# scroll-tech/scroll-prover

Measured on NVIDIA H100. Metric: chunk-proof wall-sec (degree-26 SRS: k=20+24+25 replay), lower is better.
Workload: dtype u32x8 (254-bit Montgomery integers)

## Files before the change

### scroll-prover_b200/csrc/api.cu

```cuda
#include <stdlib.h>

#include <new>

#include "common.cuh"
#include "ec.cuh"

namespace b200zk {
int32_t g1_generator_mul_run(b200zk_ctx* ctx, const Fr* scalars, uint64_t n, Affine* out);
int32_t poly_ew(b200zk_ctx* ctx, int op, Fr* r, const Fr* a, const Fr* b, const Fr& s, uint64_t n);
int32_t eval_poly(b200zk_ctx* ctx, const Fr* poly, uint64_t n, const Fr& x, Fr* out_dev);
int32_t batch_invert(b200zk_ctx* ctx, Fr* data, uint64_t n);
int32_t inner_product(b200zk_ctx* ctx, const Fr* a, const Fr* b, uint64_t n, Fr* out_dev);
int32_t kate_division(b200zk_ctx* ctx, Fr* q, const Fr* a, uint64_t n, const Fr& b);
int32_t g1_fft_run(b200zk_ctx* ctx, const void* in, bool from_jac, void* out, bool to_jac, uint32_t log_n, const Fr& omega,
                   const Fr* scale);
int32_t field_op(b200zk_ctx* ctx, int field, int op, void* r, const void* a, const void* b, uint64_t n);
}

using namespace b200zk;

#define CHECK_CTX(ctx) \
    if (!(ctx)) return B200ZK_E_INVALID

extern "C" {

int32_t b200zk_ctx_create(const int* devices, int n_devices, b200zk_ctx** out) {
    if (!out) return B200ZK_E_INVALID;
    *out = nullptr;
    if (n_devices != 1 && !(n_devices == 0 && devices == nullptr)) return B200ZK_E_UNSUPPORTED;
    int dev = (devices && n_devices == 1) ? devices[0] : 0;
    int count = 0;
    if (cudaGetDeviceCount(&count) != cudaSuccess || count == 0) {
        (void)cudaGetLastError();
        return B200ZK_E_CUDA;
    }
    if (dev < 0 || dev >= count) return B200ZK_E_INVALID;
    if (cudaSetDevice(dev) != cudaSuccess) return B200ZK_E_CUDA;
    b200zk_ctx* ctx = new (std::nothrow) b200zk_ctx();
    if (!ctx) return B200ZK_E_OOM;
    ctx->device = dev;
    cudaDeviceProp prop;
    if (cudaGetDeviceProperties(&prop, dev) == cudaSuccess) ctx->sm_count = prop.multiProcessorCount;
    if (cudaStreamCreateWithFlags(&ctx->stream, cudaStreamNonBlocking) != cudaSuccess) {
        delete ctx;
        return B200ZK_E_CUDA;
    }
    ctx->own_stream = true;
    if (const char* e = getenv("B200ZK_OVERLAP")) ctx->overlap = atoi(e);
    if (const char* e = getenv("B200ZK_ACC_L")) ctx->msm_acc_l = (uint32_t)atoi(e);
    if (const char* e = getenv("B200ZK_SCATTER_SWEEPS")) ctx->msm_scatter_sweeps = (uint32_t)atoi(e);
    if (cudaMalloc(&ctx->msm_adds_dev, 8) == cudaSuccess) cudaMemset(ctx->msm_adds_dev, 0, 8);
    else ctx->msm_adds_dev = nullptr;
    *out = ctx;
    return B200ZK_OK;
}

int32_t b200zk_ctx_destroy(b200zk_ctx* ctx) {
    CHECK_CTX(ctx);
    cudaSetDevice(ctx->device);
    cudaStreamSynchronize(ctx->stream);
    comm_destroy(ctx);
    for (Scratch* s : {&ctx->ntt_work, &ctx->stage_in, &ctx->stage_out, &ctx->msm_work, &ctx->misc})
        if (s->p) cudaFree(s->p);
    for (auto& t : ctx->tables) cudaFree(t.dev);
    if (ctx->pinned) cudaFreeHost(ctx->pinned);
    if (ctx->msm_adds_dev) cudaFree(ctx->msm_adds_dev);
    for (Scratch* s : {&ctx->colstage[0], &ctx->colstage[1], &ctx->col_coeff, &ctx->col_ext, &ctx->col_commits})
        if (s->p) cudaFree(s->p);
    for (int i = 0; i < 2; ++i) {
        if (ctx->ev_copied[i]) cudaEventDestroy(ctx->ev_copied[i]);
        if (ctx->ev_used[i]) cudaEventDestroy(ctx->ev_used[i]);
        if (ctx->ev_used_aux[i]) cudaEventDestroy(ctx->ev_used_aux[i]);
    }
    if (ctx->ev_fork) cudaEventDestroy(ctx->ev_fork);
    if (ctx->ev_join) cudaEventDestroy(ctx->ev_join);
    if (ctx->copy_stream) cudaStreamDestroy(ctx->copy_stream);
    if (ctx->aux_stream) cudaStreamDestroy(ctx->aux_stream);
    if (ctx->own_stream && ctx->stream) cudaStreamDestroy(ctx->stream);
    delete ctx;
    return B200ZK_OK;
}

const char* b200zk_last_error(const b200zk_ctx* ctx) { return ctx ? ctx->err.c_str() : "null context"; }

int32_t b200zk_ctx_set_stream(b200zk_ctx* ctx, void* cuda_stream) {
    CHECK_CTX(ctx);
    Guard g(ctx);
    B2_CUDA(ctx, cudaStreamSynchronize(ctx->stream));
    if (cuda_stream == nullptr) {
        if (!ctx->own_stream) {
            B2_CUDA(ctx, cudaStreamCreateWithFlags(&ctx->stream, cudaStreamNonBlocking));
            ctx->own_stream = true;
        }
        return B200ZK_OK;
    }
    if (ctx->own_stream && ctx->stream) cudaStreamDestroy(ctx->stream);
    ctx->stream = (cudaStream_t)cuda_stream;
    ctx->own_stream = false;
    return B200ZK_OK;
}

int32_t b200zk_ctx_synchronize(b200zk_ctx* ctx) {
    CHECK_CTX(ctx);
    Guard g(ctx);
    B2_CUDA(ctx, cudaStreamSynchronize(ctx->stream));
    return B200ZK_OK;
}

int32_t b200zk_ctx_launch_count(const b200zk_ctx* ctx, uint64_t* out) {
    if (!ctx || !out) return B200ZK_E_INVALID;
    *out = ctx->launches;
    return B200ZK_OK;
}

int32_t b200zk_buf_alloc(b200zk_ctx* ctx, uint64_t bytes, void** out_dev) {
    CHECK_CTX(ctx);
    if (!out_dev) return fail(ctx, B200ZK_E_INVALID, "buf_alloc: null out");
    Guard g(ctx);
    *out_dev = nullptr;
    cudaError_t e = cudaMalloc(out_dev, bytes ? bytes : 1);
    if (e != cudaSuccess) {
        (void)cudaGetLastError();
        return fail(ctx, B200ZK_E_OOM, "buf_alloc(%llu) failed: %s", (unsigned long long)bytes, cudaGetErrorString(e));
    }
    return B200ZK_OK;
}
int32_t b200zk_buf_free(b200zk_ctx* ctx, void* dev) {
    CHECK_CTX(ctx);
    Guard g(ctx);
    if (!dev) return B200ZK_OK;
    B2_CUDA(ctx, cudaStreamSynchronize(ctx->stream));
    B2_CUDA(ctx, cudaFree(dev));
    return B200ZK_OK;
// ... 612 lines not shown
```

### scroll-prover_b200/csrc/common.cuh

```cuda
#pragma once
#include <cuda_runtime.h>
#include <stdarg.h>
#include <stdint.h>
#include <stdio.h>
#include <string.h>

#include <mutex>
#include <string>
#include <vector>

#include "../../include/b200zk.h"
#include "ff.cuh"

namespace b200zk {

struct TwiddleTable {
    Fr omega;
    uint32_t log_n;
    Fr* dev;
};

enum ProfKey { PROF_NTT_PASS = 0, PROF_NTT_TABLE, PROF_MSM_COUNT, PROF_MSM_SCAN, PROF_MSM_SCATTER, PROF_MSM_ACCUM,
               PROF_MSM_COMBINE, PROF_MSM_REDUCE, PROF_MSM_FINISH, PROF_POLY, PROF_NKEYS };
static const char* const PROF_NAMES[PROF_NKEYS] = {"ntt_pass", "ntt_table", "msm_count", "msm_scan", "msm_scatter",
                                                   "msm_accumulate", "msm_combine", "msm_reduce", "msm_finish", "poly"};
struct ProfSpan {
    int key;
    cudaEvent_t e0, e1;
};

struct Scratch {
    void* p = nullptr;
    size_t cap = 0;
};

}

struct b200zk_srs {
    b200zk_ctx* ctx;
    void* dev_bases;
    uint64_t n;
    uint32_t tag;
    uint32_t pre_c;
    uint32_t pre_W;
};

struct b200zk_ctx {
    int device = 0;
    cudaStream_t stream = nullptr;
    bool own_stream = true;
    std::recursive_mutex mu;
    std::string err;
    uint64_t launches = 0;
    int sm_count = 132;
    b200zk::Scratch ntt_work, stage_in, stage_out, msm_work, misc;
    void* pinned = nullptr;
    size_t pinned_cap = 0;
    std::vector<b200zk::TwiddleTable> tables;
    cudaStream_t copy_stream = nullptr;
    cudaStream_t aux_stream = nullptr;
    cudaEvent_t ev_used_aux[2] = {nullptr, nullptr}, ev_fork = nullptr, ev_join = nullptr;
    int overlap = 1;
    b200zk::Scratch colstage[2], col_coeff, col_ext, col_commits;
    cudaEvent_t ev_copied[2] = {nullptr, nullptr}, ev_used[2] = {nullptr, nullptr};
    bool profiling = false;
    std::vector<b200zk::ProfSpan> prof_open;
    std::vector<cudaEvent_t> prof_pool;
    double prof_ms[b200zk::PROF_NKEYS] = {0};
    uint64_t prof_cnt[b200zk::PROF_NKEYS] = {0};
    uint32_t msm_window = 0;
    uint32_t msm_scatter_sweeps = 0;
    uint32_t msm_acc_l = 0;
    int srs_precompute = 1;
    unsigned long long* msm_adds_dev = nullptr;
    uint32_t last_c = 0, last_windows = 0;
    uint64_t last_adds = 0;
    uint32_t smem_optin = 0;
    void* nccl_comm = nullptr;
    void* comm_buf = nullptr;
    int comm_rank = 0, comm_world = 1;
};

namespace b200zk {

inline int32_t fail(b200zk_ctx* ctx, int32_t code, const char* fmt, ...) {
    char buf[512];
    va_list ap;
    va_start(ap, fmt);
    vsnprintf(buf, sizeof buf, fmt, ap);
    va_end(ap);
    if (ctx) ctx->err = buf;
    return code;
}

#define B2_CUDA(ctx, call)                                                                                   \
    do {                                                                                                     \
        cudaError_t e__ = (call);                                                                            \
        if (e__ != cudaSuccess)                                                                              \
            return ::b200zk::fail(ctx, e__ == cudaErrorMemoryAllocation ? B200ZK_E_OOM : B200ZK_E_CUDA,      \
                                  "%s failed: %s (%s:%d)", #call, cudaGetErrorString(e__), __FILE__, __LINE__); \
    } while (0)

#define B2_TRY(expr)                    \
    do {                                \
        int32_t rc__ = (expr);          \
        if (rc__ != B200ZK_OK) return rc__; \
    } while (0)

#define B2_LAUNCH_CHECK(ctx)                 \
    do {                                     \
        (ctx)->launches++;                   \
        B2_CUDA(ctx, cudaGetLastError());    \
    } while (0)

inline cudaEvent_t prof_event(b200zk_ctx* ctx) {
    if (!ctx->prof_pool.empty()) {
        cudaEvent_t e = ctx->prof_pool.back();
        ctx->prof_pool.pop_back();
        return e;
    }
    cudaEvent_t e = nullptr;
    cudaEventCreate(&e);
    return e;
}
struct ProfScope {
    b200zk_ctx* ctx;
    ProfSpan sp;
    bool on;
    ProfScope(b200zk_ctx* c, int key) : ctx(c), on(c->profiling) {
        if (!on) return;
        sp.key = key;
        sp.e0 = prof_event(c);
        sp.e1 = prof_event(c);
        cudaEventRecord(sp.e0, c->stream);
    }
    ~ProfScope() {
        if (!on) return;
        cudaEventRecord(sp.e1, ctx->stream);
        ctx->prof_open.push_back(sp);
    }
};
inline void prof_resolve(b200zk_ctx* ctx) {
    for (auto& sp : ctx->prof_open) {
        float ms = 0;
        if (cudaEventSynchronize(sp.e1) == cudaSuccess && cudaEventElapsedTime(&ms, sp.e0, sp.e1) == cudaSuccess) {
            ctx->prof_ms[sp.key] += ms;
            ctx->prof_cnt[sp.key] += 1;
        }
        ctx->prof_pool.push_back(sp.e0);
        ctx->prof_pool.push_back(sp.e1);
    }
    ctx->prof_open.clear();
}

// ... 128 lines not shown
```

### scroll-prover_b200/csrc/msm.cu

```cuda
#include "common.cuh"
#include "ec.cuh"

namespace b200zk {

static constexpr uint32_t PART_INVALID = 0x1fffffffu;
static constexpr uint32_t PART_GIANT = 0x20000000u;
static constexpr uint32_t PART_STARTS = 0x80000000u;
static constexpr uint32_t PART_ENDS = 0x40000000u;
static constexpr int MSM_MAX_BATCH = 32;
static constexpr int ACC_L_DEFAULT = 256;

struct MsmPlan {
    uint32_t c, W, B;
    uint32_t Ws;
    uint32_t batch;
    uint64_t stride;
    uint64_t NB;
};

struct MsmCols {
    const Fr* p[MSM_MAX_BATCH];
};

__device__ __forceinline__ void ld_affine(const Affine* p, Fq& x, Fq& y) {
    const uint4* q = reinterpret_cast<const uint4*>(p);
    uint4 a = __ldg(q), b = __ldg(q + 1), c = __ldg(q + 2), d = __ldg(q + 3);
    x.l.v[0] = a.x; x.l.v[1] = a.y; x.l.v[2] = a.z; x.l.v[3] = a.w;
    x.l.v[4] = b.x; x.l.v[5] = b.y; x.l.v[6] = b.z; x.l.v[7] = b.w;
    y.l.v[0] = c.x; y.l.v[1] = c.y; y.l.v[2] = c.z; y.l.v[3] = c.w;
    y.l.v[4] = d.x; y.l.v[5] = d.y; y.l.v[6] = d.z; y.l.v[7] = d.w;
}

__global__ void __launch_bounds__(256) msm_count(MsmCols cols, uint64_t n, MsmPlan pl, uint32_t* hist, uint32_t* digits_all) {
    const uint32_t col = blockIdx.y;
    const Fr* scalars = cols.p[0];
#pragma unroll
    for (int q = 1; q < MSM_MAX_BATCH; ++q)
        if (q == (int)col) scalars = cols.p[q];
    uint32_t* digits = digits_all + (uint64_t)col * pl.W * n;
    uint32_t* hist_c = hist + (uint64_t)col * pl.Ws * pl.B;
    uint64_t stride = (uint64_t)gridDim.x * blockDim.x;
    for (uint64_t i = (uint64_t)blockIdx.x * blockDim.x + threadIdx.x; i < n; i += stride) {
        Fr s = scalars[i];
        if (s.is_zero()) {
            for (uint32_t w = 0; w < pl.W; ++w) digits[(uint64_t)w * n + i] = 0;
            continue;
        }
        s = s.from_mont();
        uint32_t l[8];
#pragma unroll
        for (int k = 0; k < 8; ++k) l[k] = s.l.v[k];
        const uint32_t c = pl.c, mask = (1u << c) - 1, half = 1u << (c - 1);
        uint32_t carry = 0;
        for (uint32_t w = 0; w < pl.W; ++w) {
            uint32_t v = (l[0] & mask) + carry;
#pragma unroll
            for (int k = 0; k < 7; ++k) l[k] = __funnelshift_r(l[k], l[k + 1], c);
            l[7] >>= c;
            uint32_t enc;
            if (v > half) {
                enc = (1u << c) - v;
                carry = 1;
                if (enc) enc |= 0x80000000u;
            } else {
                enc = v;
                carry = 0;
            }
            digits[(uint64_t)w * n + i] = enc;
            if (enc) atomicAdd(&hist_c[(pl.Ws == 1 ? 0ull : (uint64_t)w * pl.B) + (enc & 0x7fffffffu) - 1], 1u);
        }
    }
}

__global__ void __launch_bounds__(256) msm_scatter(const uint32_t* __restrict__ digits, uint64_t n, MsmPlan pl,
                                                   uint32_t* cursor, uint32_t* entries, const uint32_t* __restrict__ total_entries,
                                                   uint32_t sweep, uint32_t max_sweeps) {
    uint32_t eff = 1;
    if (max_sweeps > 1) {
        uint64_t bytes = 4ull * (*total_entries);
        eff = (uint32_t)((bytes + (1ull << 28) - 1) >> 28);
        eff = eff < 1 ? 1 : (eff > max_sweeps ? max_sweeps : eff);
    }
    if (sweep >= eff) return;
    const uint32_t b_lo = eff == 3 ? (pl.B / 3) * sweep : (pl.B / eff) * sweep;
    const uint32_t b_hi = (sweep + 1 == eff) ? pl.B : (eff == 3 ? (pl.B / 3) * (sweep + 1) : (pl.B / eff) * (sweep + 1));
    const uint32_t cw = blockIdx.y;
    const uint32_t col = cw / pl.W, w = cw - col * pl.W;
    const uint32_t* dg = digits + (uint64_t)cw * n;
    uint32_t* cur = cursor + ((uint64_t)col * pl.Ws + (pl.Ws == 1 ? 0u : w)) * pl.B;
    const uint32_t woff = (uint32_t)((uint64_t)w * pl.stride);
    uint64_t stride = (uint64_t)gridDim.x * blockDim.x;
    for (uint64_t i = (uint64_t)blockIdx.x * blockDim.x + threadIdx.x; i < n; i += stride) {
        uint32_t d = dg[i];
        if (!d) continue;
        uint32_t bk = (d & 0x7fffffffu) - 1;
        if (bk < b_lo || bk >= b_hi) continue;
        uint32_t pos = atomicAdd(&cur[bk], 1u);
        entries[pos] = ((uint32_t)i + woff) | (d & 0x80000000u);
    }
}

static constexpr int SCAN_TPB = 256, SCAN_ITEMS = 16, SCAN_TILE = SCAN_TPB * SCAN_ITEMS;

__device__ __forceinline__ uint32_t block_exclusive_scan(uint32_t v, uint32_t* total) {
    __shared__ uint32_t warp_sums[SCAN_TPB / 32];
    uint32_t lane = threadIdx.x & 31, wid = threadIdx.x >> 5;
    uint32_t x = v;
#pragma unroll
    for (int o = 1; o < 32; o <<= 1) {
        uint32_t y = __shfl_up_sync(0xffffffffu, x, o);
        if (lane >= (uint32_t)o) x += y;
    }
    if (lane == 31) warp_sums[wid] = x;
    __syncthreads();
    if (wid == 0) {
        uint32_t s = (lane < SCAN_TPB / 32) ? warp_sums[lane] : 0;
#pragma unroll
        for (int o = 1; o < 32; o <<= 1) {
            uint32_t y = __shfl_up_sync(0xffffffffu, s, o);
            if (lane >= (uint32_t)o) s += y;
        }
        if (lane < SCAN_TPB / 32) warp_sums[lane] = s;
    }
    __syncthreads();
    uint32_t warp_off = wid ? warp_sums[wid - 1] : 0;
    *total = warp_sums[SCAN_TPB / 32 - 1];
    uint32_t r = warp_off + x - v;
    __syncthreads();
    return r;
}

__global__ void __launch_bounds__(SCAN_TPB) scan_tile_sums(const uint32_t* in, uint64_t n, uint32_t* tile_sums) {
    uint64_t base = (uint64_t)blockIdx.x * SCAN_TILE + (uint64_t)threadIdx.x * SCAN_ITEMS;
    uint32_t s = 0;
#pragma unroll
    for (int k = 0; k < SCAN_ITEMS; ++k)
        if (base + k < n) s += in[base + k];
    uint32_t total;
    block_exclusive_scan(s, &total);
    if (threadIdx.x == 0) tile_sums[blockIdx.x] = total;
}
__global__ void __launch_bounds__(SCAN_TPB) scan_tile_offsets(uint32_t* tile_sums, uint32_t ntiles, uint32_t* grand_total,
                                                              unsigned long long* running) {
    uint32_t carry = 0;
    for (uint32_t base = 0; base < ntiles; base += SCAN_TPB) {
        uint32_t i = base + threadIdx.x;
        uint32_t v = i < ntiles ? tile_sums[i] : 0, total;
        uint32_t ex = block_exclusive_scan(v, &total);
        if (i < ntiles) tile_sums[i] = carry + ex;
        carry += total;
    }
    if (threadIdx.x == 0) {
        *grand_total = carry;
        if (running) atomicAdd(running, (unsigned long long)carry);
    }
}
__global__ void __launch_bounds__(SCAN_TPB) scan_apply(const uint32_t* in, uint64_t n, const uint32_t* tile_offs, uint32_t* out,
                                                     uint32_t* out2) {
    uint64_t base = (uint64_t)blockIdx.x * SCAN_TILE + (uint64_t)threadIdx.x * SCAN_ITEMS;
    uint32_t v[SCAN_ITEMS], s = 0;
#pragma unroll
    for (int k = 0; k < SCAN_ITEMS; ++k) {
        v[k] = (base + k < n) ? in[base + k] : 0;
        s += v[k];
    }
    uint32_t total;
    uint32_t off = block_exclusive_scan(s, &total) + tile_offs[blockIdx.x];
#pragma unroll
    for (int k = 0; k < SCAN_ITEMS; ++k) {
        if (base + k < n) {
            out[base + k] = off;
            out2[base + k] = off;
        }
        off += v[k];
    }
}

__device__ __forceinline__ void st_xyzz(XYZZ* p, const XYZZ& v) {
    uint4* q = reinterpret_cast<uint4*>(p);
    const Fq* f = &v.x;
#pragma unroll
    for (int k = 0; k < 4; ++k) {
        q[2 * k] = make_uint4(f[k].l.v[0], f[k].l.v[1], f[k].l.v[2], f[k].l.v[3]);
        q[2 * k + 1] = make_uint4(f[k].l.v[4], f[k].l.v[5], f[k].l.v[6], f[k].l.v[7]);
    }
}
__device__ __forceinline__ XYZZ ld_xyzz(const XYZZ* p) {
    const uint4* q = reinterpret_cast<const uint4*>(p);
    XYZZ v;
    Fq* f = &v.x;
#pragma unroll
    for (int k = 0; k < 4; ++k) {
        uint4 a = q[2 * k], b = q[2 * k + 1];
        f[k].l.v[0] = a.x; f[k].l.v[1] = a.y; f[k].l.v[2] = a.z; f[k].l.v[3] = a.w;
        f[k].l.v[4] = b.x; f[k].l.v[5] = b.y; f[k].l.v[6] = b.z; f[k].l.v[7] = b.w;
    }
    return v;
}

__global__ void __launch_bounds__(256, 2)
msm_accumulate(const Affine* __restrict__ bases, const uint32_t* __restrict__ entries, const uint32_t* __restrict__ offsets,
               uint64_t NB, XYZZ* __restrict__ buckets, uint32_t* __restrict__ part_id, XYZZ* __restrict__ part_val,
               uint64_t nthreads, uint32_t* __restrict__ giant_flag, uint32_t ACC_L) {
    uint64_t tau = (uint64_t)blockIdx.x * blockDim.x + threadIdx.x;
    if (tau >= nthreads) return;
    const uint32_t M = offsets[NB];
    const uint32_t BIG_BUCKET = 4 * ACC_L;
    uint64_t start = tau * ACC_L;
    part_id[2 * tau] = PART_INVALID;
    part_id[2 * tau + 1] = PART_INVALID;
    if (start >= M) return;
    uint32_t end = (start + ACC_L < M) ? (uint32_t)(start + ACC_L) : M;
    uint64_t lo = 0, hi = NB;
    while (hi - lo > 1) {
        uint64_t mid = (lo + hi) >> 1;
        if (offsets[mid] <= start) lo = mid; else hi = mid;
    }
    uint32_t b = (uint32_t)lo;
    uint32_t bucket_start = offsets[b], bucket_end = offsets[b + 1];
    bool run_starts = (bucket_start == (uint32_t)start);
    uint32_t slot = 0;
    XYZZ acc = XYZZ::identity();
    uint32_t pos = (uint32_t)start;
    while (true) {
        bool at_end = (pos == end);
        if (at_end || pos == bucket_end) {
            bool run_ends = (pos == bucket_end);
            if (run_starts && run_ends) {
                st_xyzz(buckets + b, acc);
            } else {
                uint32_t giant = (bucket_end - bucket_start > BIG_BUCKET) ? PART_GIANT : 0u;
                if (giant) *giant_flag = 1u;
                part_id[2 * tau + slot] = b | giant | (run_starts ? PART_STARTS : 0u) | (run_ends ? PART_ENDS : 0u);
                st_xyzz(part_val + 2 * tau + slot, acc);
                ++slot;
            }
            if (at_end) break;
            acc = XYZZ::identity();
            bucket_start = pos;
            do { ++b; bucket_end = offsets[b + 1]; } while (bucket_end == pos);
            run_starts = true;
        }
        uint32_t e = entries[pos];
        Fq px, py;
        ld_affine(bases + (e & 0x7fffffffu), px, py);
        if (!(px.is_zero() && py.is_zero())) {
            if (e & 0x80000000u) py = py.neg();
            xyzz_madd(acc, px, py);
        }
        ++pos;
    }
}

__global__ void __launch_bounds__(128) msm_combine_heads(const uint32_t* __restrict__ part_id, const XYZZ* __restrict__ part_val,
                                                         uint64_t nrec, XYZZ* __restrict__ buckets) {
    uint64_t r = (uint64_t)blockIdx.x * blockDim.x + threadIdx.x;
    if (r >= nrec) return;
    uint32_t id = part_id[r];
    if ((id & PART_INVALID) == PART_INVALID || (id & PART_GIANT) || !(id & PART_STARTS)) return;
// ... 195 lines not shown
}

static uint32_t pick_window(uint64_t n) {
    if (n < 32) return n < 4 ? 2 : 4;
    double best = 1e300;
    uint32_t bc = 8;
    for (uint32_t c = 5; c <= 23; ++c) {
        uint32_t W = 254 / c + 1;
        if ((double)n * W >= 4.0e9) continue;
        double cost = (double)n * W * 10.0 + (double)W * (double)(1ull << c) * 40.0 + (double)W * 4096.0;
        if (cost < best) {
            best = cost;
            bc = c;
        }
    }
    return bc;
}

static size_t align_up(size_t v, size_t a) { return (v + a - 1) / a * a; }

__global__ void __launch_bounds__(128) srs_shift_kernel(const Affine* __restrict__ in, Affine* __restrict__ out, uint64_t n, uint32_t c) {
    uint64_t i = (uint64_t)blockIdx.x * blockDim.x + threadIdx.x;
    if (i >= n) return;
    Affine a = in[i];
    XYZZ p = xyzz_from_affine(a);
    for (uint32_t d = 0; d < c; ++d) p = xyzz_dbl(p);
    out[i] = xyzz_to_affine(p);
}

static uint32_t pick_window_precomputed(uint64_t n) {
    double best = 1e300;
    uint32_t bc = 10;
    for (uint32_t c = 8; c <= 23; ++c) {
        uint32_t W = 254 / c + 1;
        if ((double)n * W >= 2.0e9) continue;
        double cost = (double)n * W * 10.0 + (double)(1ull << c) * 40.0;
        if (cost < best) {
            best = cost;
            bc = c;
        }
    }
    return bc;
}

static int32_t srs_precompute_run(b200zk_ctx* ctx, Affine* tables, uint64_t n, uint32_t c, uint32_t W) {
    for (uint32_t w = 1; w < W; ++w) {
        srs_shift_kernel<<<(uint32_t)((n + 127) / 128), 128, 0, ctx->stream>>>(tables + (uint64_t)(w - 1) * n, tables + (uint64_t)w * n, n, c);
        B2_LAUNCH_CHECK(ctx);
    }
    return B200ZK_OK;
}

static uint32_t msm_max_batch(uint64_t n, uint32_t pre_c) {
    uint32_t c = pre_c ? pre_c : pick_window(n);
    uint64_t per_col = (n ? n : 1) * (254 / c + 1);
    uint64_t b = (1ull << 28) / per_col;
    return (uint32_t)(b < 1 ? 1 : (b > MSM_MAX_BATCH ? MSM_MAX_BATCH : b));
}

static int32_t msm_run_batch(b200zk_ctx* ctx, const Affine* bases, const Fr* const* cols, uint32_t batch, uint64_t n, Jacobian* out_dev,
                             uint32_t pre_c, uint64_t pre_stride) {
    if (n >= (1ull << 31)) return fail(ctx, B200ZK_E_UNSUPPORTED, "msm: n = %llu >= 2^31", (unsigned long long)n);
    if (batch < 1 || batch > (uint32_t)MSM_MAX_BATCH) return fail(ctx, B200ZK_E_INVALID, "msm: batch %u out of range [1,%d]", batch, MSM_MAX_BATCH);
    MsmPlan pl;
    pl.c = pre_c ? pre_c : (ctx->msm_window ? ctx->msm_window : pick_window(n));
    if (pl.c < 2 || pl.c > 24) return fail(ctx, B200ZK_E_INVALID, "msm: window %u out of range [2,24]", pl.c);
    pl.W = 254 / pl.c + 1;
    pl.B = 1u << (pl.c - 1);
    pl.Ws = pre_c ? 1 : pl.W;
    pl.batch = batch;
    pl.stride = pre_c ? pre_stride : 0;
    pl.NB = (uint64_t)batch * pl.Ws * pl.B;
    uint64_t max_entries = n * pl.W * batch;
    if (max_entries >= 0xffffffffull) return fail(ctx, B200ZK_E_UNSUPPORTED, "msm: n*W*batch too large for window %u", pl.c);
    MsmCols colp;
    for (int q = 0; q < MSM_MAX_BATCH; ++q) colp.p[q] = cols[q < (int)batch ? q : 0];
    ctx->last_c = pl.c;
    ctx->last_windows = pl.W;
    ctx->last_adds = n * pl.W;

    const uint32_t ACC_L = ctx->msm_acc_l ? ctx->msm_acc_l : (uint32_t)ACC_L_DEFAULT;
    uint64_t nthreads = (max_entries + ACC_L - 1) / ACC_L;
    if (nthreads == 0) nthreads = 1;
    uint32_t ntiles = (uint32_t)((pl.NB + SCAN_TILE - 1) / SCAN_TILE);
    size_t off = 0;
    auto carve = [&](size_t bytes) { size_t o = off; off = align_up(off + bytes, 256); return o; };
    size_t o_hist = carve(4 * (pl.NB + 1)), o_offs = carve(4 * (pl.NB + 1)), o_cursor = carve(4 * (pl.NB + 1));
    size_t o_tiles = carve(4 * (size_t)(ntiles + 1));
    size_t o_flag = carve(256);
    size_t o_entries = carve(4 * (max_entries + 4));
    size_t o_digits = carve(4 * (max_entries + 4));
    size_t o_buckets = carve(sizeof(XYZZ) * pl.NB);
    size_t o_pid = carve(4 * 2 * nthreads), o_pval = carve(sizeof(XYZZ) * 2 * nthreads);
    uint64_t nthreads2 = (2 * nthreads + COMBINE_LR - 1) / COMBINE_LR;
    size_t o_pid2 = carve(4 * 2 * nthreads2), o_pval2 = carve(sizeof(XYZZ) * 2 * nthreads2);
    const uint32_t kc = pl.c / 2;
    const uint32_t red_cols = 1u << kc, red_rows = pl.B >> kc;
    const uint32_t sets = batch * pl.Ws;
    size_t red_len = (size_t)sets * (red_rows + red_cols);
    uint32_t q_max = 0;
    while ((1u << q_max) < (red_rows > red_cols ? red_rows : red_cols)) ++q_max;
    size_t o_gr = carve(sizeof(XYZZ) * red_len), o_sums = carve(sizeof(XYZZ) * 2 * (q_max + 1) * sets);
    B2_TRY(scratch_reserve(ctx, ctx->msm_work, off));
    char* base = (char*)ctx->msm_work.p;
    uint32_t* hist = (uint32_t*)(base + o_hist);
    uint32_t* offsets = (uint32_t*)(base + o_offs);
    uint32_t* cursor = (uint32_t*)(base + o_cursor);
    uint32_t* tiles = (uint32_t*)(base + o_tiles);
    uint32_t* giant_flag = (uint32_t*)(base + o_flag);
    uint32_t* entries = (uint32_t*)(base + o_entries);
    uint32_t* digits = (uint32_t*)(base + o_digits);
    uint32_t* pid2 = (uint32_t*)(base + o_pid2);
    XYZZ* pval2 = (XYZZ*)(base + o_pval2);
    XYZZ* buckets = (XYZZ*)(base + o_buckets);
    uint32_t* pid = (uint32_t*)(base + o_pid);
    XYZZ* pval = (XYZZ*)(base + o_pval);
    XYZZ* grpR = (XYZZ*)(base + o_gr);
    XYZZ* red_sums = (XYZZ*)(base + o_sums);

    cudaStream_t st = ctx->stream;
    B2_CUDA(ctx, cudaMemsetAsync(hist, 0, 4 * (pl.NB + 1), st));
    B2_CUDA(ctx, cudaMemsetAsync(giant_flag, 0, 4, st));
    B2_CUDA(ctx, cudaMemsetAsync(buckets, 0, sizeof(XYZZ) * pl.NB, st));
    uint32_t sblocks = (uint32_t)ctx->sm_count * 8;
    if (n) {
        uint64_t want = (n + 255) / 256;
        uint32_t per_col = (sblocks + batch - 1) / batch;
        uint32_t blocks = (uint32_t)(want < per_col ? want : per_col);
        {
            ProfScope ps_(ctx, PROF_MSM_COUNT);
            msm_count<<<dim3(blocks, batch), 256, 0, st>>>(colp, n, pl, hist, digits);
        }
        B2_LAUNCH_CHECK(ctx);
    }
    {
        ProfScope ps_(ctx, PROF_MSM_SCAN);
        scan_tile_sums<<<ntiles, SCAN_TPB, 0, st>>>(hist, pl.NB, tiles);
        B2_LAUNCH_CHECK(ctx);
        scan_tile_offsets<<<1, SCAN_TPB, 0, st>>>(tiles, ntiles, offsets + pl.NB, ctx->msm_adds_dev);
        B2_LAUNCH_CHECK(ctx);
        scan_apply<<<ntiles, SCAN_TPB, 0, st>>>(hist, pl.NB, tiles, offsets, cursor);
        B2_LAUNCH_CHECK(ctx);
    }
    if (n) {
        {
            ProfScope ps_(ctx, PROF_MSM_SCATTER);
            uint64_t want = (n + 1023) / 1024;
            uint32_t blocks = (uint32_t)(want < 0x7fffffffull ? (want ? want : 1) : 0x7fffffffull);
            {
                uint32_t sweeps = 1;
                if (pl.Ws == 1 && batch == 1) {
                    uint64_t region = 200ull << 20;
                    sweeps = (uint32_t)((4 * max_entries + region - 1) / region);
                    if (sweeps < 1) sweeps = 1;
                    if (sweeps > 4) sweeps = 4;
                    if (ctx->msm_scatter_sweeps) sweeps = ctx->msm_scatter_sweeps;
                }
                for (uint32_t sw = 0; sw < sweeps; ++sw) {
                    uint32_t bx = blocks;
                    if (sw > 0) {
                        uint32_t lean = (uint32_t)ctx->sm_count * 32u / (batch * pl.W) + 1;
                        if (lean < bx) bx = lean;
                    }
                    msm_scatter<<<dim3(bx, batch * pl.W), 256, 0, st>>>(digits, n, pl, cursor, entries, offsets + pl.NB, sw, sweeps);
                    if (sw + 1 < sweeps) B2_LAUNCH_CHECK(ctx);
                }
            }
        }
        B2_LAUNCH_CHECK(ctx);
        uint32_t ablocks = (uint32_t)((nthreads + 255) / 256);
        {
            ProfScope ps_(ctx, PROF_MSM_ACCUM);
            msm_accumulate<<<ablocks, 256, 0, st>>>(bases, entries, offsets, pl.NB, buckets, pid, pval, nthreads, giant_flag, ACC_L);
        }
        B2_LAUNCH_CHECK(ctx);
        {
            ProfScope ps_(ctx, PROF_MSM_COMBINE);
            uint64_t nrec = 2 * nthreads;
            msm_combine_heads<<<(uint32_t)((nrec + 127) / 128), 128, 0, st>>>(pid, pval, nrec, buckets);
            B2_LAUNCH_CHECK(ctx);
            uint32_t *in_id = pid, *out_id = pid2;
            XYZZ *in_val = pval, *out_val = pval2;
            while (nrec > 2048) {
                uint64_t nt = (nrec + COMBINE_LR - 1) / COMBINE_LR;
                msm_combine_level<<<(uint32_t)((nt + 127) / 128), 128, 0, st>>>(in_id, in_val, nrec, buckets, out_id, out_val, nt, giant_flag);
                B2_LAUNCH_CHECK(ctx);
                nrec = 2 * nt;
                uint32_t* ti = in_id; in_id = out_id; out_id = ti;
                XYZZ* tv = in_val; in_val = out_val; out_val = tv;
            }
            msm_combine_final<<<(uint32_t)((nrec + 127) / 128), 128, 0, st>>>(in_id, in_val, nrec, buckets, giant_flag);
            B2_LAUNCH_CHECK(ctx);
        }
    }
    {
        ProfScope ps_(ctx, PROF_MSM_REDUCE);
        msm_rowcol_sums<<<dim3(red_rows + red_cols, sets), RED_T, 0, st>>>(buckets, pl.B, kc, grpR);
        B2_LAUNCH_CHECK(ctx);
        msm_bit_sums<<<dim3(q_max + 1, 2, sets), RED_T, 0, st>>>(grpR, pl.B, kc, q_max, red_sums);
        B2_LAUNCH_CHECK(ctx);
        msm_finish<<<batch, 64, 0, st>>>(pl, kc, q_max, red_sums, out_dev);
        B2_LAUNCH_CHECK(ctx);
    }
    return B200ZK_OK;
}

int32_t msm_bases(b200zk_ctx* ctx, const Affine* bases, const Fr* scalars, uint64_t n, Jacobian* out_dev) {
    return msm_run_batch(ctx, bases, &scalars, 1, n, out_dev, 0, 0);
}

int32_t srs_init(b200zk_ctx* ctx, b200zk_srs* s, const void* g1_affine) {
    const uint64_t n = s->n;
    s->dev_bases = nullptr;
    s->pre_c = 0;
    s->pre_W = 1;
    size_t bytes = sizeof(Affine) * (n ? n : 1);
    if (ctx->srs_precompute && n >= (1ull << 16)) {
        uint32_t c = pick_window_precomputed(n), W = 254 / c + 1;
        size_t free_b = 0, total_b = 0;
        if (cudaMemGetInfo(&free_b, &total_b) == cudaSuccess && (double)bytes * W < 0.35 * (double)free_b) {
            s->pre_c = c;
            s->pre_W = W;
            bytes *= W;
        }
    }
    cudaError_t e = cudaMalloc(&s->dev_bases, bytes);
    if (e != cudaSuccess) {
        (void)cudaGetLastError();
        s->dev_bases = nullptr;
        return fail(ctx, B200ZK_E_OOM, "srs_register: cudaMalloc(%zu) failed", bytes);
    }
    cudaMemcpyKind kind = is_device_ptr(g1_affine) ? cudaMemcpyDeviceToDevice : cudaMemcpyHostToDevice;
    e = n ? cudaMemcpyAsync(s->dev_bases, g1_affine, sizeof(Affine) * n, kind, ctx->stream) : cudaSuccess;
    if (e == cudaSuccess) e = cudaStreamSynchronize(ctx->stream);
    if (e != cudaSuccess) {
        srs_free(s);
        return fail(ctx, B200ZK_E_CUDA, "srs_register: upload failed: %s", cudaGetErrorString(e));
    }
    if (s->pre_c) {
        int32_t rc = srs_precompute_run(ctx, (Affine*)s->dev_bases, n, s->pre_c, s->pre_W);
        if (rc == B200ZK_OK && cudaStreamSynchronize(ctx->stream) != cudaSuccess) rc = B200ZK_E_CUDA;
        if (rc != B200ZK_OK) {
            srs_free(s);
            return fail(ctx, rc, "srs_register: precomputation failed");
        }
    }
    return B200ZK_OK;
}

void srs_free(b200zk_srs* s) {
    if (s->dev_bases) cudaFree(s->dev_bases);
    s->dev_bases = nullptr;
// ... 30 lines not shown
```

Baseline: 4.536.

## Replace MSM global-atomic histogram and scatter with two-level tiled bucket sort

Swaps the global-atomic bucket histogram and the multi-sweep scatter in the MSM for a two-level bin sort. Per-tile shared-memory counts go into a bin-by-tile matrix, which is prefix-scanned. Entries are placed into coarse bins in a staging buffer, then each bin is sorted into final buckets in shared memory with dynamic bin assignment. The goal is to cut contended global atomics and random scattered writes. In exchange it adds extra passes, a staging buffer, heavy shared-memory use, and a new failure path when no plan fits.

```diff
diff --git a/scroll-prover_b200/csrc/api.cu b/scroll-prover_b200/csrc/api.cu
--- a/scroll-prover_b200/csrc/api.cu
+++ b/scroll-prover_b200/csrc/api.cu
@@ -48,7 +48,6 @@
     ctx->own_stream = true;
     if (const char* e = getenv("B200ZK_OVERLAP")) ctx->overlap = atoi(e);
     if (const char* e = getenv("B200ZK_ACC_L")) ctx->msm_acc_l = (uint32_t)atoi(e);
-    if (const char* e = getenv("B200ZK_SCATTER_SWEEPS")) ctx->msm_scatter_sweeps = (uint32_t)atoi(e);
     if (cudaMalloc(&ctx->msm_adds_dev, 8) == cudaSuccess) cudaMemset(ctx->msm_adds_dev, 0, 8);
     else ctx->msm_adds_dev = nullptr;
     *out = ctx;
diff --git a/scroll-prover_b200/csrc/common.cuh b/scroll-prover_b200/csrc/common.cuh
--- a/scroll-prover_b200/csrc/common.cuh
+++ b/scroll-prover_b200/csrc/common.cuh
@@ -69,7 +69,6 @@
     double prof_ms[b200zk::PROF_NKEYS] = {0};
     uint64_t prof_cnt[b200zk::PROF_NKEYS] = {0};
     uint32_t msm_window = 0;
-    uint32_t msm_scatter_sweeps = 0;
     uint32_t msm_acc_l = 0;
     int srs_precompute = 1;
     unsigned long long* msm_adds_dev = nullptr;
diff --git a/scroll-prover_b200/csrc/msm.cu b/scroll-prover_b200/csrc/msm.cu
--- a/scroll-prover_b200/csrc/msm.cu
+++ b/scroll-prover_b200/csrc/msm.cu
@@ -31,16 +31,106 @@
     y.l.v[4] = d.x; y.l.v[5] = d.y; y.l.v[6] = d.z; y.l.v[7] = d.w;
 }
 
-__global__ void __launch_bounds__(256) msm_count(MsmCols cols, uint64_t n, MsmPlan pl, uint32_t* hist, uint32_t* digits_all) {
-    const uint32_t col = blockIdx.y;
+static constexpr int SCAN_TPB = 256, SCAN_ITEMS = 16, SCAN_TILE = SCAN_TPB * SCAN_ITEMS;
+
+template <int TPB = SCAN_TPB>
+__device__ __forceinline__ uint32_t block_exclusive_scan(uint32_t v, uint32_t* total) {
+    static_assert(TPB % 32 == 0 && TPB <= 1024, "one warp scans the warp sums");
+    __shared__ uint32_t warp_sums[TPB / 32];
+    uint32_t lane = threadIdx.x & 31, wid = threadIdx.x >> 5;
+    uint32_t x = v;
+#pragma unroll
+    for (int o = 1; o < 32; o <<= 1) {
+        uint32_t y = __shfl_up_sync(0xffffffffu, x, o);
+        if (lane >= (uint32_t)o) x += y;
+    }
+    if (lane == 31) warp_sums[wid] = x;
+    __syncthreads();
+    if (wid == 0) {
+        uint32_t s = (lane < TPB / 32) ? warp_sums[lane] : 0;
+#pragma unroll
+        for (int o = 1; o < 32; o <<= 1) {
+            uint32_t y = __shfl_up_sync(0xffffffffu, s, o);
+            if (lane >= (uint32_t)o) s += y;
+        }
+        if (lane < TPB / 32) warp_sums[lane] = s;
+    }
+    __syncthreads();
+    uint32_t warp_off = wid ? warp_sums[wid - 1] : 0;
+    *total = warp_sums[TPB / 32 - 1];
+    uint32_t r = warp_off + x - v;
+    __syncthreads();
+    return r;
+}
+
+__global__ void __launch_bounds__(SCAN_TPB) scan_tile_sums(const uint32_t* in, uint64_t n, uint32_t* tile_sums) {
+    uint64_t base = (uint64_t)blockIdx.x * SCAN_TILE + (uint64_t)threadIdx.x * SCAN_ITEMS;
+    uint32_t s = 0;
+#pragma unroll
+    for (int k = 0; k < SCAN_ITEMS; ++k)
+        if (base + k < n) s += in[base + k];
+    uint32_t total;
+    block_exclusive_scan(s, &total);
+    if (threadIdx.x == 0) tile_sums[blockIdx.x] = total;
+}
+__global__ void __launch_bounds__(SCAN_TPB) scan_tile_offsets(uint32_t* tile_sums, uint32_t ntiles, uint32_t* grand_total,
+                                                              unsigned long long* running) {
+    uint32_t carry = 0;
+    for (uint32_t base = 0; base < ntiles; base += SCAN_TPB) {
+        uint32_t i = base + threadIdx.x;
+        uint32_t v = i < ntiles ? tile_sums[i] : 0, total;
+        uint32_t ex = block_exclusive_scan(v, &total);
+        if (i < ntiles) tile_sums[i] = carry + ex;
+        carry += total;
+    }
+    if (threadIdx.x == 0) {
+        *grand_total = carry;
+        if (running) atomicAdd(running, (unsigned long long)carry);
+    }
+}
+__global__ void __launch_bounds__(SCAN_TPB) scan_apply(const uint32_t* in, uint64_t n, const uint32_t* tile_offs, uint32_t* out) {
+    uint64_t base = (uint64_t)blockIdx.x * SCAN_TILE + (uint64_t)threadIdx.x * SCAN_ITEMS;
+    uint32_t v[SCAN_ITEMS], s = 0;
+#pragma unroll
+    for (int k = 0; k < SCAN_ITEMS; ++k) {
+        v[k] = (base + k < n) ? in[base + k] : 0;
+        s += v[k];
+    }
+    uint32_t total;
+    uint32_t off = block_exclusive_scan(s, &total) + tile_offs[blockIdx.x];
+#pragma unroll
+    for (int k = 0; k < SCAN_ITEMS; ++k) {
+        if (base + k < n) out[base + k] = off;
+        off += v[k];
+    }
+}
+
+static constexpr int BIN_TPB = 1024;
+static constexpr int SORT_U = 4;
+
+struct BinPlan {
+    uint32_t S;
+    uint32_t t;
+    uint32_t wbits;
+    uint32_t fcol;
+    uint32_t tiles;
+    uint32_t nbins;
+};
+
+__global__ void __launch_bounds__(BIN_TPB) msm_bin_count(MsmCols cols, uint64_t n, MsmPlan pl, BinPlan bp, uint32_t* __restrict__ mat,
+                                                     uint32_t* __restrict__ digits_all) {
+    extern __shared__ uint32_t bin_cnt[];
+    const uint32_t col = blockIdx.y, tile = blockIdx.x;
     const Fr* scalars = cols.p[0];
 #pragma unroll
     for (int q = 1; q < MSM_MAX_BATCH; ++q)
         if (q == (int)col) scalars = cols.p[q];
     uint32_t* digits = digits_all + (uint64_t)col * pl.W * n;
-    uint32_t* hist_c = hist + (uint64_t)col * pl.Ws * pl.B;
-    uint64_t stride = (uint64_t)gridDim.x * blockDim.x;
-    for (uint64_t i = (uint64_t)blockIdx.x * blockDim.x + threadIdx.x; i < n; i += stride) {
+    for (uint32_t k = threadIdx.x; k < bp.fcol; k += blockDim.x) bin_cnt[k] = 0;
+    __syncthreads();
+    const uint64_t i0 = (uint64_t)tile << bp.t, i1 = (i0 + (1ull << bp.t) < n) ? i0 + (1ull << bp.t) : n;
+    const uint32_t c = pl.c, mask = (1u << c) - 1, half = 1u << (c - 1);
+    for (uint64_t i = i0 + threadIdx.x; i < i1; i += blockDim.x) {
         Fr s = scalars[i];
         if (s.is_zero()) {
             for (uint32_t w = 0; w < pl.W; ++w) digits[(uint64_t)w * n + i] = 0;
@@ -50,7 +140,6 @@
         uint32_t l[8];
 #pragma unroll
         for (int k = 0; k < 8; ++k) l[k] = s.l.v[k];
-        const uint32_t c = pl.c, mask = (1u << c) - 1, half = 1u << (c - 1);
         uint32_t carry = 0;
         for (uint32_t w = 0; w < pl.W; ++w) {
             uint32_t v = (l[0] & mask) + carry;
@@ -67,114 +156,149 @@
                 carry = 0;
             }
             digits[(uint64_t)w * n + i] = enc;
-            if (enc) atomicAdd(&hist_c[(pl.Ws == 1 ? 0ull : (uint64_t)w * pl.B) + (enc & 0x7fffffffu) - 1], 1u);
-        }
-    }
-}
-
-__global__ void __launch_bounds__(256) msm_scatter(const uint32_t* __restrict__ digits, uint64_t n, MsmPlan pl,
-                                                   uint32_t* cursor, uint32_t* entries, const uint32_t* __restrict__ total_entries,
-                                                   uint32_t sweep, uint32_t max_sweeps) {
-    uint32_t eff = 1;
-    if (max_sweeps > 1) {
-        uint64_t bytes = 4ull * (*total_entries);
-        eff = (uint32_t)((bytes + (1ull << 28) - 1) >> 28);
-        eff = eff < 1 ? 1 : (eff > max_sweeps ? max_sweeps : eff);
-    }
-    if (sweep >= eff) return;
-    const uint32_t b_lo = eff == 3 ? (pl.B / 3) * sweep : (pl.B / eff) * sweep;
-    const uint32_t b_hi = (sweep + 1 == eff) ? pl.B : (eff == 3 ? (pl.B / 3) * (sweep + 1) : (pl.B / eff) * (sweep + 1));
-    const uint32_t cw = blockIdx.y;
-    const uint32_t col = cw / pl.W, w = cw - col * pl.W;
-    const uint32_t* dg = digits + (uint64_t)cw * n;
-    uint32_t* cur = cursor + ((uint64_t)col * pl.Ws + (pl.Ws == 1 ? 0u : w)) * pl.B;
-    const uint32_t woff = (uint32_t)((uint64_t)w * pl.stride);
-    uint64_t stride = (uint64_t)gridDim.x * blockDim.x;
-    for (uint64_t i = (uint64_t)blockIdx.x * blockDim.x + threadIdx.x; i < n; i += stride) {
-        uint32_t d = dg[i];
-        if (!d) continue;
-        uint32_t bk = (d & 0x7fffffffu) - 1;
-        if (bk < b_lo || bk >= b_hi) continue;
-        uint32_t pos = atomicAdd(&cur[bk], 1u);
-        entries[pos] = ((uint32_t)i + woff) | (d & 0x80000000u);
-    }
-}
-
-static constexpr int SCAN_TPB = 256, SCAN_ITEMS = 16, SCAN_TILE = SCAN_TPB * SCAN_ITEMS;
-
-__device__ __forceinline__ uint32_t block_exclusive_scan(uint32_t v, uint32_t* total) {
-    __shared__ uint32_t warp_sums[SCAN_TPB / 32];
-    uint32_t lane = threadIdx.x & 31, wid = threadIdx.x >> 5;
-    uint32_t x = v;
-#pragma unroll
-    for (int o = 1; o < 32; o <<= 1) {
-        uint32_t y = __shfl_up_sync(0xffffffffu, x, o);
-        if (lane >= (uint32_t)o) x += y;
-    }
-    if (lane == 31) warp_sums[wid] = x;
+            if (enc) atomicAdd(&bin_cnt[((pl.Ws == 1 ? 0u : w * pl.B) + (enc & 0x7fffffffu) - 1) >> bp.S], 1u);
+        }
+    }
     __syncthreads();
-    if (wid == 0) {
-        uint32_t s = (lane < SCAN_TPB / 32) ? warp_sums[lane] : 0;
-#pragma unroll
-        for (int o = 1; o < 32; o <<= 1) {
-            uint32_t y = __shfl_up_sync(0xffffffffu, s, o);
-            if (lane >= (uint32_t)o) s += y;
-        }
-        if (lane < SCAN_TPB / 32) warp_sums[lane] = s;
-    }
+    uint32_t* row = mat + (uint64_t)col * bp.fcol * bp.tiles + tile;
+    for (uint32_t k = threadIdx.x; k < bp.fcol; k += blockDim.x) row[(uint64_t)k * bp.tiles] = bin_cnt[k];
+}
+
+__global__ void __launch_bounds__(BIN_TPB) msm_bin_place(const uint32_t* __restrict__ digits_all, uint64_t n, MsmPlan pl, BinPlan bp,
+                                                     const uint32_t* __restrict__ mat, uint32_t* __restrict__ staging) {
+    extern __shared__ uint32_t cur[];
+    const uint32_t Wp = pl.Ws == 1 ? 1u : pl.W, cw = blockIdx.y, col = cw / Wp, wp = cw - col * Wp, tile = blockIdx.x;
+    const uint32_t nloc = pl.B >> bp.S;
+    const uint64_t bin0 = (uint64_t)col * bp.fcol + (uint64_t)wp * nloc;
+    for (uint32_t k = threadIdx.x; k < nloc; k += blockDim.x) cur[k] = mat[(bin0 + k) * bp.tiles + tile];
     __syncthreads();
-    uint32_t warp_off = wid ? warp_sums[wid - 1] : 0;
-    *total = warp_sums[SCAN_TPB / 32 - 1];
-    uint32_t r = warp_off + x - v;
-    __syncthreads();
-    return r;
-}
-
-__global__ void __launch_bounds__(SCAN_TPB) scan_tile_sums(const uint32_t* in, uint64_t n, uint32_t* tile_sums) {
-    uint64_t base = (uint64_t)blockIdx.x * SCAN_TILE + (uint64_t)threadIdx.x * SCAN_ITEMS;
-    uint32_t s = 0;
-#pragma unroll
-    for (int k = 0; k < SCAN_ITEMS; ++k)
-        if (base + k < n) s += in[base + k];
-    uint32_t total;
-    block_exclusive_scan(s, &total);
-    if (threadIdx.x == 0) tile_sums[blockIdx.x] = total;
-}
-__global__ void __launch_bounds__(SCAN_TPB) scan_tile_offsets(uint32_t* tile_sums, uint32_t ntiles, uint32_t* grand_total,
-                                                              unsigned long long* running) {
-    uint32_t carry = 0;
-    for (uint32_t base = 0; base < ntiles; base += SCAN_TPB) {
-        uint32_t i = base + threadIdx.x;
-        uint32_t v = i < ntiles ? tile_sums[i] : 0, total;
-        uint32_t ex = block_exclusive_scan(v, &total);
-        if (i < ntiles) tile_sums[i] = carry + ex;
-        carry += total;
-    }
-    if (threadIdx.x == 0) {
-        *grand_total = carry;
-        if (running) atomicAdd(running, (unsigned long long)carry);
-    }
-}
-__global__ void __launch_bounds__(SCAN_TPB) scan_apply(const uint32_t* in, uint64_t n, const uint32_t* tile_offs, uint32_t* out,
-                                                     uint32_t* out2) {
-    uint64_t base = (uint64_t)blockIdx.x * SCAN_TILE + (uint64_t)threadIdx.x * SCAN_ITEMS;
-    uint32_t v[SCAN_ITEMS], s = 0;
-#pragma unroll
-    for (int k = 0; k < SCAN_ITEMS; ++k) {
-        v[k] = (base + k < n) ? in[base + k] : 0;
-        s += v[k];
-    }
-    uint32_t total;
-    uint32_t off = block_exclusive_scan(s, &total) + tile_offs[blockIdx.x];
-#pragma unroll
-    for (int k = 0; k < SCAN_ITEMS; ++k) {
-        if (base + k < n) {
-            out[base + k] = off;
-            out2[base + k] = off;
-        }
-        off += v[k];
-    }
-}
+    const uint64_t i0 = (uint64_t)tile << bp.t, i1 = (i0 + (1ull << bp.t) < n) ? i0 + (1ull << bp.t) : n;
+    const uint32_t low_mask = (1u << bp.S) - 1, sh_w = bp.S + 1, sh_i = bp.wbits + bp.S + 1;
+    const uint32_t w_end = pl.Ws == 1 ? pl.W : wp + 1;
+    for (uint32_t w = pl.Ws == 1 ? 0u : wp; w < w_end; ++w) {
+        const uint32_t* dg = digits_all + ((uint64_t)col * pl.W + w) * n;
+        for (uint64_t i = i0 + threadIdx.x; i < i1; i += SORT_U * BIN_TPB) {
+            uint32_t d[SORT_U];
+#pragma unroll
+            for (int u = 0; u < SORT_U; ++u) d[u] = i + u * BIN_TPB < i1 ? dg[i + u * BIN_TPB] : 0u;
+#pragma unroll
+            for (int u = 0; u < SORT_U; ++u) {
+                if (!d[u]) continue;
+                const uint32_t b = (d[u] & 0x7fffffffu) - 1;
+                const uint32_t pos = atomicAdd(&cur[b >> bp.S], 1u);
+                staging[pos] = ((uint32_t)(i + u * BIN_TPB - i0) << sh_i) | (bp.wbits ? w << sh_w : 0u) | ((b & low_mask) << 1) |
+                               (d[u] >> 31);
+            }
+        }
+    }
+}
+
+__global__ void __launch_bounds__(BIN_TPB) msm_bin_sort(const uint32_t* __restrict__ mat, const uint32_t* __restrict__ total,
+                                                    const uint32_t* __restrict__ staging, MsmPlan pl, BinPlan bp,
+                                                    uint32_t* __restrict__ offsets, uint32_t* __restrict__ entries,
+                                                    uint32_t* __restrict__ next_bin, uint32_t cap) {
+    extern __shared__ uint32_t sort_sh[];
+    __shared__ uint32_t bin_sh;
+    const uint32_t nb = 1u << bp.S, per = (nb + BIN_TPB - 1) / BIN_TPB;
+    uint32_t* cnt = sort_sh;
+    uint32_t* run = sort_sh + nb;
+    uint32_t* out = run + bp.tiles + 1;
+    const uint32_t low_mask = nb - 1, sh_w = bp.S + 1, sh_i = bp.wbits + bp.S + 1, w_mask = (1u << bp.wbits) - 1;
+    const uint32_t stride = (uint32_t)pl.stride;
+    while (true) {
+        if (threadIdx.x == 0) bin_sh = atomicAdd(next_bin, 1u);
+        __syncthreads();
+        const uint32_t bin = bin_sh;
+        if (bin >= bp.nbins) return;
+        const uint32_t* r = mat + (uint64_t)bin * bp.tiles;
+        for (uint32_t k = threadIdx.x; k < bp.tiles; k += blockDim.x) run[k] = r[k];
+        if (threadIdx.x == 0) run[bp.tiles] = bin + 1 < bp.nbins ? r[bp.tiles] : *total;
+        for (uint32_t k = threadIdx.x; k < nb; k += blockDim.x) cnt[k] = 0;
+        __syncthreads();
+        const uint32_t lo = run[0], hi = run[bp.tiles];
+        const bool fits = hi - lo <= cap;
+        for (uint64_t p0 = lo + threadIdx.x; p0 < hi; p0 += SORT_U * BIN_TPB) {
+            uint32_t x[SORT_U];
+#pragma unroll
+            for (int u = 0; u < SORT_U; ++u) x[u] = p0 + u * BIN_TPB < hi ? staging[p0 + u * BIN_TPB] : 0u;
+#pragma unroll
+            for (int u = 0; u < SORT_U; ++u)
+                if (p0 + u * BIN_TPB < hi) atomicAdd(&cnt[(x[u] >> 1) & low_mask], 1u);
+        }
+        __syncthreads();
+        const uint32_t k0 = threadIdx.x * per;
+        uint32_t sum = 0;
+        for (uint32_t j = 0; j < per; ++j)
+            if (k0 + j < nb) sum += cnt[k0 + j];
+        uint32_t tot;
+        uint32_t ex = block_exclusive_scan<BIN_TPB>(sum, &tot) + lo;
+        for (uint32_t j = 0; j < per; ++j)
+            if (k0 + j < nb) {
+                const uint32_t v = cnt[k0 + j];
+                cnt[k0 + j] = ex;
+                offsets[(uint64_t)bin * nb + k0 + j] = ex;
+                ex += v;
+            }
+        __syncthreads();
+        for (uint64_t p0 = lo + threadIdx.x; p0 < hi; p0 += SORT_U * BIN_TPB) {
+            uint32_t x[SORT_U];
+#pragma unroll
+            for (int u = 0; u < SORT_U; ++u) x[u] = p0 + u * BIN_TPB < hi ? staging[p0 + u * BIN_TPB] : 0u;
+#pragma unroll
+            for (int u = 0; u < SORT_U; ++u) {
+                const uint64_t p = p0 + u * BIN_TPB;
+                if (p >= hi) break;
+                uint32_t a = 0, z = bp.tiles;
+                while (z - a > 1) {
+                    const uint32_t m = (a + z) >> 1;
+                    if (run[m] <= p) a = m; else z = m;
+                }
+                uint32_t e = (a << bp.t) + (x[u] >> sh_i);
+                if (bp.wbits) e += ((x[u] >> sh_w) & w_mask) * stride;
+                const uint32_t pos = atomicAdd(&cnt[(x[u] >> 1) & low_mask], 1u);
+                if (fits) out[pos - lo] = e | (x[u] << 31);
+                else entries[pos] = e | (x[u] << 31);
+            }
+        }
+        __syncthreads();
+        if (fits)
+            for (uint32_t k = threadIdx.x; k < hi - lo; k += blockDim.x) entries[lo + k] = out[k];
+        __syncthreads();
+    }
+}
+
+static bool bin_plan(const MsmPlan& pl, uint64_t n, uint32_t sms, BinPlan* bp) {
+    uint32_t wbits = 0, ln = 0, lsb = 0;
+    if (pl.Ws == 1)
+        while ((1u << wbits) < pl.W) ++wbits;
+    while ((1ull << ln) < n) ++ln;
+    const uint64_t set_b = (uint64_t)pl.Ws * pl.B;
+    while ((1ull << lsb) < set_b) ++lsb;
+    const uint32_t s_max = pl.c - 1 < 14 ? pl.c - 1 : 14, s_min = lsb > 15 ? lsb - 15 : 0;
+    uint32_t S = 0;
+    while (S < s_max && (double)n * pl.W * (double)(2ull << S) <= 8192.0 * (double)set_b) ++S;
+    if (S < s_min) S = s_min;
+    for (;; --S) {
+        uint32_t t_lo = ln > 12 ? ln - 12 : 0;
+        if (ln > S + 5 && ln - S - 5 > t_lo) t_lo = ln - S - 5;
+        const uint32_t t_hi = 31 - wbits - S;
+        uint32_t t = 17;
+        while (t > 8 && (uint64_t)pl.batch * ((n + (1ull << t) - 1) >> t) < 2ull * sms) --t;
+        if (t < t_lo) t = t_lo;
+        if (t > t_hi) t = t_hi;
+        if (t >= t_lo) {
+            bp->S = S;
+            bp->t = t;
+            bp->wbits = wbits;
+            bp->fcol = (uint32_t)(set_b >> S);
+            bp->tiles = (uint32_t)((n + (1ull << t) - 1) >> t);
+            bp->nbins = pl.batch * bp->fcol;
+            return true;
+        }
+        if (S == s_min) return false;
+    }
+}
+
 
 __device__ __forceinline__ void st_xyzz(XYZZ* p, const XYZZ& v) {
     uint4* q = reinterpret_cast<uint4*>(p);
@@ -536,14 +660,18 @@
     const uint32_t ACC_L = ctx->msm_acc_l ? ctx->msm_acc_l : (uint32_t)ACC_L_DEFAULT;
     uint64_t nthreads = (max_entries + ACC_L - 1) / ACC_L;
     if (nthreads == 0) nthreads = 1;
-    uint32_t ntiles = (uint32_t)((pl.NB + SCAN_TILE - 1) / SCAN_TILE);
+    BinPlan bp;
+    if (!bin_plan(pl, n, (uint32_t)ctx->sm_count, &bp))
+        return fail(ctx, B200ZK_E_UNSUPPORTED, "msm: no bucket-sort plan for n = %llu, window %u", (unsigned long long)n, pl.c);
+    const uint64_t mat_len = (uint64_t)bp.nbins * bp.tiles;
+    const uint32_t ntiles = (uint32_t)((mat_len + SCAN_TILE - 1) / SCAN_TILE);
     size_t off = 0;
     auto carve = [&](size_t bytes) { size_t o = off; off = align_up(off + bytes, 256); return o; };
-    size_t o_hist = carve(4 * (pl.NB + 1)), o_offs = carve(4 * (pl.NB + 1)), o_cursor = carve(4 * (pl.NB + 1));
+    size_t o_offs = carve(4 * (pl.NB + 1));
     size_t o_tiles = carve(4 * (size_t)(ntiles + 1));
     size_t o_flag = carve(256);
     size_t o_entries = carve(4 * (max_entries + 4));
-    size_t o_digits = carve(4 * (max_entries + 4));
+    size_t o_staging = carve(4 * (max_entries + 4));
     size_t o_buckets = carve(sizeof(XYZZ) * pl.NB);
     size_t o_pid = carve(4 * 2 * nthreads), o_pval = carve(sizeof(XYZZ) * 2 * nthreads);
     uint64_t nthreads2 = (2 * nthreads + COMBINE_LR - 1) / COMBINE_LR;
@@ -557,71 +685,63 @@
     size_t o_gr = carve(sizeof(XYZZ) * red_len), o_sums = carve(sizeof(XYZZ) * 2 * (q_max + 1) * sets);
     B2_TRY(scratch_reserve(ctx, ctx->msm_work, off));
     char* base = (char*)ctx->msm_work.p;
-    uint32_t* hist = (uint32_t*)(base + o_hist);
     uint32_t* offsets = (uint32_t*)(base + o_offs);
-    uint32_t* cursor = (uint32_t*)(base + o_cursor);
     uint32_t* tiles = (uint32_t*)(base + o_tiles);
     uint32_t* giant_flag = (uint32_t*)(base + o_flag);
+    uint32_t* next_bin = giant_flag + 1;
     uint32_t* entries = (uint32_t*)(base + o_entries);
-    uint32_t* digits = (uint32_t*)(base + o_digits);
+    uint32_t* staging = (uint32_t*)(base + o_staging);
     uint32_t* pid2 = (uint32_t*)(base + o_pid2);
     XYZZ* pval2 = (XYZZ*)(base + o_pval2);
     XYZZ* buckets = (XYZZ*)(base + o_buckets);
+    uint32_t* mat = (uint32_t*)buckets;
     uint32_t* pid = (uint32_t*)(base + o_pid);
     XYZZ* pval = (XYZZ*)(base + o_pval);
     XYZZ* grpR = (XYZZ*)(base + o_gr);
     XYZZ* red_sums = (XYZZ*)(base + o_sums);
 
     cudaStream_t st = ctx->stream;
-    B2_CUDA(ctx, cudaMemsetAsync(hist, 0, 4 * (pl.NB + 1), st));
-    B2_CUDA(ctx, cudaMemsetAsync(giant_flag, 0, 4, st));
-    B2_CUDA(ctx, cudaMemsetAsync(buckets, 0, sizeof(XYZZ) * pl.NB, st));
-    uint32_t sblocks = (uint32_t)ctx->sm_count * 8;
+    B2_CUDA(ctx, cudaMemsetAsync(giant_flag, 0, 8, st));
     if (n) {
-        uint64_t want = (n + 255) / 256;
-        uint32_t per_col = (sblocks + batch - 1) / batch;
-        uint32_t blocks = (uint32_t)(want < per_col ? want : per_col);
+        const uint32_t nb = 1u << bp.S, cap = 28160u - nb - bp.tiles - 1;
+        const size_t tile_smem = 4 * (size_t)bp.fcol, sort_smem = 4 * ((size_t)nb + bp.tiles + 1 + cap);
+        if (!(ctx->smem_optin & (1u << 9))) {
+            const int most = 160 * 1024;
+            B2_CUDA(ctx, cudaFuncSetAttribute(msm_bin_count, cudaFuncAttributeMaxDynamicSharedMemorySize, most));
+            B2_CUDA(ctx, cudaFuncSetAttribute(msm_bin_place, cudaFuncAttributeMaxDynamicSharedMemorySize, most));
+            B2_CUDA(ctx, cudaFuncSetAttribute(msm_bin_sort, cudaFuncAttributeMaxDynamicSharedMemorySize, most));
+            ctx->smem_optin |= 1u << 9;
+        }
+        const dim3 tgrid(bp.tiles, batch);
         {
             ProfScope ps_(ctx, PROF_MSM_COUNT);
-            msm_count<<<dim3(blocks, batch), 256, 0, st>>>(colp, n, pl, hist, digits);
+            msm_bin_count<<<tgrid, BIN_TPB, tile_smem, st>>>(colp, n, pl, bp, mat, entries);
         }
         B2_LAUNCH_CHECK(ctx);
-    }
-    {
-        ProfScope ps_(ctx, PROF_MSM_SCAN);
-        scan_tile_sums<<<ntiles, SCAN_TPB, 0, st>>>(hist, pl.NB, tiles);
+        {
+            ProfScope ps_(ctx, PROF_MSM_SCAN);
+            scan_tile_sums<<<ntiles, SCAN_TPB, 0, st>>>(mat, mat_len, tiles);
+            B2_LAUNCH_CHECK(ctx);
+            scan_tile_offsets<<<1, SCAN_TPB, 0, st>>>(tiles, ntiles, offsets + pl.NB, ctx->msm_adds_dev);
+            B2_LAUNCH_CHECK(ctx);
+            scan_apply<<<ntiles, SCAN_TPB, 0, st>>>(mat, mat_len, tiles, mat);
+            B2_LAUNCH_CHECK(ctx);
+        }
+        {
+            ProfScope ps_(ctx, PROF_MSM_COUNT);
+            const uint32_t Wp = pl.Ws == 1 ? 1u : pl.W;
+            msm_bin_place<<<dim3(bp.tiles, batch * Wp), BIN_TPB, 4 * (size_t)(pl.B >> bp.S), st>>>(entries, n, pl, bp, mat, staging);
+        }
         B2_LAUNCH_CHECK(ctx);
-        scan_tile_offsets<<<1, SCAN_TPB, 0, st>>>(tiles, ntiles, offsets + pl.NB, ctx->msm_adds_dev);
-        B2_LAUNCH_CHECK(ctx);
-        scan_apply<<<ntiles, SCAN_TPB, 0, st>>>(hist, pl.NB, tiles, offsets, cursor);
-        B2_LAUNCH_CHECK(ctx);
-    }
-    if (n) {
         {
             ProfScope ps_(ctx, PROF_MSM_SCATTER);
-            uint64_t want = (n + 1023) / 1024;
-            uint32_t blocks = (uint32_t)(want < 0x7fffffffull ? (want ? want : 1) : 0x7fffffffull);
-            {
-                uint32_t sweeps = 1;
-                if (pl.Ws == 1 && batch == 1) {
-                    uint64_t region = 200ull << 20;
-                    sweeps = (uint32_t)((4 * max_entries + region - 1) / region);
-                    if (sweeps < 1) sweeps = 1;
-                    if (sweeps > 4) sweeps = 4;
-                    if (ctx->msm_scatter_sweeps) sweeps = ctx->msm_scatter_sweeps;
-                }
-                for (uint32_t sw = 0; sw < sweeps; ++sw) {
-                    uint32_t bx = blocks;
-                    if (sw > 0) {
-                        uint32_t lean = (uint32_t)ctx->sm_count * 32u / (batch * pl.W) + 1;
-                        if (lean < bx) bx = lean;
-                    }
-                    msm_scatter<<<dim3(bx, batch * pl.W), 256, 0, st>>>(digits, n, pl, cursor, entries, offsets + pl.NB, sw, sweeps);
-                    if (sw + 1 < sweeps) B2_LAUNCH_CHECK(ctx);
-                }
-            }
+            const uint32_t most = 2 * (uint32_t)ctx->sm_count, sblocks = bp.nbins < most ? bp.nbins : most;
+            msm_bin_sort<<<sblocks, BIN_TPB, sort_smem, st>>>(mat, offsets + pl.NB, staging, pl, bp, offsets, entries, next_bin, cap);
         }
         B2_LAUNCH_CHECK(ctx);
+    }
+    B2_CUDA(ctx, cudaMemsetAsync(buckets, 0, sizeof(XYZZ) * pl.NB, st));
+    if (n) {
         uint32_t ablocks = (uint32_t)((nthreads + 255) / 256);
         {
             ProfScope ps_(ctx, PROF_MSM_ACCUM);
```

Result: no change. 4.531, median of 6 (-0.1%).
